# neggles/neurosis

Hardware: AMD Instinct MI355X
Metric: train images/sec (node) SDXL 1024^2 (higher is better)
Workload: dtype bf16

## Files before the change

### include/neurosis_hip.h

```cpp
#ifndef NEUROSIS_HIP_H
#define NEUROSIS_HIP_H

#ifdef __cplusplus
extern "C" {
#endif

const char* nk_last_error(void);
int nk_abi_version(void);

int nk_linear_fwd(const void* x, const void* w, const float* bias, const void* residual, void* y,
                  int M, int N, int K, long ldx, long ldw, long ldr, long ldy, float alpha, void* stream);
int nk_linear_dgrad(const void* dy, const void* w, const void* dx_add, void* dx, int M, int N, int K,
                    long lddy, long ldw, long ldadd, long lddx, void* stream);
long nk_linear_fwd_geglu_ok(int M, int I, int K);
int nk_linear_fwd_geglu(const void* x, const void* w, const float* bias, void* u, void* h, int M, int I, int K, long ldx, long ldw, long ldu,
                        long ldh, void* stream);
int nk_linear_dgrad_geglu(const void* dy, const void* w, const void* u, void* du, int M, int N, int I, long lddy, long ldw, long ldu,
                          long lddu, void* stream);
int nk_linear_fwd_geglu_s(const void* x, const void* w, const float* bias, void* s, void* h, int M, int I, int K, long ldx, long ldw, long lds,
                          long ldh, void* stream);
int nk_linear_dgrad_geglu_s(const void* dy, const void* w, const void* s, void* du, int M, int N, int I, long lddy, long ldw, long lds,
                            long lddu, void* stream);
int nk_linear_wgrad(const void* dy, const void* x, float* dw, int M, int N, int K, long lddy, long ldx,
                    long lddw, int accumulate, void* stream);
int nk_linear_wgrad_bias(const void* dy, const void* x, float* dw, float* dbias, int M, int N, int K, long lddy, long ldx, long lddw,
                         int accumulate, void* stream);

int nk_gemm_sk_status(void);

int nk_health_status(void);
int nk_health_clear(void);
int nk_health_export(int* dst, void* stream);
int nk_health_import(const int* src, void* stream);
int nk_debug_raise_health(void* stream);
int nk_debug_stamp(unsigned long long* dst, void* stream);
int nk_debug_launch_log(int mode);
long nk_debug_launch_names(char* buf, long cap);
// ... 241 lines not shown
```

### neurosis_amd/csrc/gemm.hip

```cpp
#include "nk_common.h"
#include "nk_gemm.h"
#include "gemm_plan.h"

#define NTHREADS 256
#define KC_IMAGE_BYTES (128 * 128)
#define MC_ROW_BYTES (128 * 2 + 16)
#define MC_IMAGE_BYTES (BK * MC_ROW_BYTES)
#define OPND_BYTES MC_IMAGE_BYTES
#define STAGE_BYTES (2 * OPND_BYTES)
#define SMEM_BYTES (2 * STAGE_BYTES)

static_assert(SMEM_BYTES >= BM * CS_LD * 4, "epilogue staging must fit");

__device__ __forceinline__ bool is_kc(int mode) { return mode == OP_KC || mode == OP_KCG; }

__device__ __forceinline__ long gather_offset(const NkGather& g, int n, int bh, int bw, int kh, int kw,
                                              int c, bool& valid) {
  int hn = bh + kh * g.ks;
  int wn = bw + kw * g.ks;
  bool ok = (hn >= 0) & (wn >= 0);
  ok &= (((hn | wn) & g.need_even) == 0);
  const int sh = g.div >> 1;
  int h = hn >> sh, w = wn >> sh;
  ok &= (h < g.H) & (w < g.W);
// ... 1148 lines not shown
        for (int j = 0; j < NJ; ++j)
          acc[i][j] = __builtin_amdgcn_mfma_f32_16x16x32_bf16(bfr[j], af[i], acc[i][j], 0, 0, 0);
    }
  }
#pragma unroll
  for (int ib = 0; ib < MI / 4; ++ib)
#pragma unroll
    for (int half = 0; half < NJ / 2; ++half) {
      float4_t pair[4][2];
#pragma unroll
      for (int i = 0; i < 4; ++i) { pair[i][0] = acc[ib * 4 + i][2 * half]; pair[i][1] = acc[ib * 4 + i][2 * half + 1]; }
      reg_epilogue_64x32<0>(p, p.C, pair, m0 + wm * WM + ib * 64, n0 + wn * WN + half * 32, lane);
    }
}

template <int AMODE, int GEGLU = 0>
__global__ __launch_bounds__(512, 2) void nk_gemm_xl2g_kernel(const NkGemmParams p) {
  extern __shared__ __attribute__((aligned(16))) char smem[];
  const int tid = threadIdx.x, lane = tid & 63, wave = tid >> 6;
  const int wm = wave >> 2, wn = wave & 3;
  const int nwg = gridDim.x, bid = blockIdx.x;
  const int q8 = nwg >> 3, r8 = nwg & 7, xcd = bid & 7;
  const int wg = (xcd < r8 ? xcd * (q8 + 1) : r8 * (q8 + 1) + (xcd - r8) * q8) + (bid >> 3);
  const int ntn = (p.N + XL_BN - 1) / XL_BN, ntm = (p.M + XL_BM - 1) / XL_BM;
  constexpr int GM = 4;
  const int per_group = GM * ntn;
  const int group = wg / per_group;
  const int first_m = group * GM;
  const int gm = min(GM, ntm - first_m);
  const int in_group = wg - group * per_group;
  const int nt = in_group / gm;
  const int m0 = (first_m + (in_group - nt * gm)) * XL_BM, n0 = nt * XL_BN;
  const int kend = p.K, nk = (p.K + BK - 1) / BK;

  OperandDMA<AMODE, 2> a0, a1;
  OperandDMA<OP_KC, 2> b0, b1;
  a0.init(p.A, p.lda, p.M, m0, tid, p.ga);
  a1.init(p.A, p.lda, p.M, m0 + 128, tid, p.ga);
  if constexpr (GEGLU) {
    const int I = p.N >> 1, wv = tid >> 6;
    const int gb0 = wv, gb1 = 8 + wv;
    b0.init(p.B, p.ldb, p.N, ((gb0 & 1) ? I : 0) + (n0 >> 1) + (gb0 >> 1) * 16 - wv * 16, tid, p.gb);
    b1.init(p.B, p.ldb, p.N, ((gb1 & 1) ? I : 0) + (n0 >> 1) + (gb1 >> 1) * 16 - wv * 16, tid, p.gb);
  } else {
    b0.init(p.B, p.ldb, p.N, n0, tid, p.gb);
    b1.init(p.B, p.ldb, p.N, n0 + 128, tid, p.gb);
  }
  const int s0 = p.k_rotate ? (xcd * nk) >> 3 : 0;
  const int wrap_at = nk - s0;
  int na0 = 0, na1 = 0, nb0 = 0, nb1 = 0, ka0 = kend, ka1 = kend, kb0 = kend, kb1 = kend;
  a0.start(s0 * BK); a1.start(s0 * BK); b0.start(s0 * BK); b1.start(s0 * BK);
#define X2_NEXT(op, src, g, cnt, ke)                        \
  do {                                                      \
    op.next_sources(ke, src, g, p.tw);                      \
    if (++cnt == wrap_at) { op.start(0); ke = s0 * BK; }    \
  } while (0)
#define X2_ISSUE(op, img, g, cnt, ke)                       \
  do {                                                      \
    const bf16_t* s_[2];                                    \
    X2_NEXT(op, s_, g, cnt, ke);                            \
    op.fire(0, s_[0], img); op.fire(1, s_[1], img);         \
  } while (0)
  float4_t acc[8][4];
#pragma unroll
  for (int i = 0; i < 8; ++i)
#pragma unroll
    for (int j = 0; j < 4; ++j) acc[i][j] = (float4_t){0.f, 0.f, 0.f, 0.f};

  bf16x8_t ar[8], bc0[4], bc1[4];
  typedef __attribute__((address_space(3))) const char* lds_c;
  const unsigned lds0 = (unsigned)(size_t)(lds_c)smem;
  const unsigned x0 = (unsigned)(((lane >> 4) ^ (lane & 7)) << 4);
  const unsigned arow = lds0 + (unsigned)(wm * 128 + (lane & 15)) * 128u;
  const unsigned brow = lds0 + 32768u + (unsigned)(wn * 64 + (lane & 15)) * 128u;
  const unsigned a_k0 = arow + x0, a_k1 = arow + (x0 ^ 64u), b_k0 = brow + x0, b_k1 = brow + (x0 ^ 64u);
#define X2_RD1(f, addr, OFF) asm volatile("ds_read_b128 %0, %1 offset:%2" : "=v"(f) : "v"(addr), "n"((OFF)))
#define X2_RDA(half)                                                                                             \
  X2_RD1(ar[0], ca0, (half) * 8192); X2_RD1(ar[1], ca0, (half) * 8192 + 2048); X2_RD1(ar[2], ca0, (half) * 8192 + 4096);    \
  X2_RD1(ar[3], ca0, (half) * 8192 + 6144); X2_RD1(ar[4], ca1, (half) * 8192); X2_RD1(ar[5], ca1, (half) * 8192 + 2048);    \
  X2_RD1(ar[6], ca1, (half) * 8192 + 4096); X2_RD1(ar[7], ca1, (half) * 8192 + 6144)
#define X2_RDB(f, half)                                                                                          \
  X2_RD1(f[0], cb0, (half) * 4096); X2_RD1(f[1], cb0, (half) * 4096 + 2048); X2_RD1(f[2], cb1, (half) * 4096);              \
  X2_RD1(f[3], cb1, (half) * 4096 + 2048)
#define X2_BAR() __builtin_amdgcn_sched_barrier(0); __builtin_amdgcn_s_barrier(); __builtin_amdgcn_sched_barrier(0)
#define X2_MM(rb, cb, bf, PREP)                                                                                  \
  asm volatile("s_waitcnt lgkmcnt(0)" ::: "memory");                                                             \
  __builtin_amdgcn_sched_barrier(0);                                                                             \
  __builtin_amdgcn_s_setprio(1);                                                                                 \
  PREP;               \
  _Pragma("unroll") for (int ks = 0; ks < 2; ++ks)                                                               \
    _Pragma("unroll") for (int i = 0; i < 4; ++i)                                                                \
      _Pragma("unroll") for (int j = 0; j < 2; ++j)                                                              \
        acc[(rb) + i][(cb) + j] = __builtin_amdgcn_mfma_f32_16x16x32_bf16(bf[ks * 2 + j], ar[ks * 4 + i], acc[(rb) + i][(cb) + j], 0, 0, 0); \
  __builtin_amdgcn_s_setprio(0)

  const bf16_t* sa0[2];
  const bf16_t* sa1[2];
  const bf16_t* sb0[2];
  const bf16_t* sb1[2];
  if (nk > 0) {
    X2_ISSUE(a0, smem, p.ga, na0, ka0);
    X2_ISSUE(a1, smem + 16384, p.ga, na1, ka1);
    X2_ISSUE(b0, smem + 32768, p.gb, nb0, kb0);
    X2_ISSUE(b1, smem + 49152, p.gb, nb1, kb1);
    X2_ISSUE(b0, smem + XL_STAGE_BYTES + 32768, p.gb, nb0, kb0);
    X2_ISSUE(b1, smem + XL_STAGE_BYTES + 49152, p.gb, nb1, kb1);
    asm volatile("s_waitcnt vmcnt(4)" ::: "memory");
  }
  X2_NEXT(a1, sa1, p.ga, na1, ka1);
  X2_BAR();
  if (wm == 1) { X2_BAR(); }
  for (int t = 0; t < nk; ++t) {
    const unsigned so = (unsigned)(t & 1) * XL_STAGE_BYTES;
    char* cur = smem + so;
// ... 15 lines not shown
    X2_BAR();
    X2_RDA(1);
    X2_BAR();
    X2_MM(4, 2, bc1, X2_NEXT(b0, sb0, p.gb, nb0, kb0); X2_NEXT(b1, sb1, p.gb, nb1, kb1));
    X2_BAR();
    b0.fire(0, sb0[0], cur + 32768);
    b0.fire(1, sb0[1], cur + 32768);
    b1.fire(0, sb1[0], cur + 49152);
    b1.fire(1, sb1[1], cur + 49152);
    asm volatile("s_waitcnt vmcnt(4)" ::: "memory");
    X2_BAR();
    X2_MM(4, 0, bc0, X2_NEXT(a1, sa1, p.ga, na1, ka1));
    X2_BAR();
  }
  if (wm == 0) { X2_BAR(); }
  asm volatile("s_waitcnt vmcnt(0)" ::: "memory");
#undef X2_NEXT
#undef X2_ISSUE
#undef X2_RD1
#undef X2_RDA
#undef X2_RDB
#undef X2_BAR
#undef X2_MM
  if constexpr (GEGLU) {
    const int I = p.N >> 1;
    const int abase = (n0 >> 1) + wn * 32;
    const int cl = (lane >> 4) * 4;
    float4_t ba[2], bg[2];
#pragma unroll
    for (int q = 0; q < 2; ++q) {
      ba[q] = p.bias ? *(const float4_t*)(p.bias + abase + q * 16 + cl) : (float4_t){0.f, 0.f, 0.f, 0.f};
      bg[q] = p.bias ? *(const float4_t*)(p.bias + I + abase + q * 16 + cl) : (float4_t){0.f, 0.f, 0.f, 0.f};
    }
    NkGemmParams ph = p;
    ph.N = I; ph.ldc = p.ld_h; ph.bias = nullptr;
    NkGemmParams ps = p;
    ps.bias = nullptr;
#pragma unroll
    for (int ib = 0; ib < 2; ++ib) {
      float4_t pa[4][2], pg[4][2], phh[4][2];
#pragma unroll
      for (int i = 0; i < 4; ++i)
#pragma unroll
        for (int q = 0; q < 2; ++q) {
          pa[i][q] = acc[ib * 4 + i][2 * q];
          pg[i][q] = acc[ib * 4 + i][2 * q + 1];
#pragma unroll
          for (int r = 0; r < 4; ++r) {
            const float av = bf2f(f2bf(pa[i][q][r] + ba[q][r])), gv = bf2f(f2bf(pg[i][q][r] + bg[q][r]));
            float cdf, pdf;
            normal_cdf_pdf(gv, cdf, pdf);
            const float ge = gv * cdf;
            phh[i][q][r] = av * ge;
            if (p.geglu_save) {
              pa[i][q][r] = ge;
              pg[i][q][r] = av * (cdf + gv * pdf);
            }
          }
        }
      const int mb = m0 + wm * 128 + ib * 64;
      if (p.geglu_save) {
        reg_epilogue_64x32<0>(ps, p.C, pa, mb, abase, lane);
        reg_epilogue_64x32<0>(ps, p.C, pg, mb, I + abase, lane);
      } else {
        reg_epilogue_64x32<0>(p, p.C, pa, mb, abase, lane);
        reg_epilogue_64x32<0>(p, p.C, pg, mb, I + abase, lane);
      }
      reg_epilogue_64x32<0>(ph, p.geglu_h, phh, mb, abase, lane);
    }
    return;
  }
#pragma unroll
  for (int ib = 0; ib < 2; ++ib)
#pragma unroll
    for (int half = 0; half < 2; ++half) {
      float4_t pair[4][2];
#pragma unroll
      for (int i = 0; i < 4; ++i) { pair[i][0] = acc[ib * 4 + i][2 * half]; pair[i][1] = acc[ib * 4 + i][2 * half + 1]; }
      reg_epilogue_64x32<0>(p, p.C, pair, m0 + wm * 128 + ib * 64, n0 + wn * 64 + half * 32, lane);
    }
}

__global__ void nk_zero_f32_kernel(float* __restrict__ dst, size_t n);
#include "gemm_g2.h"
#include "gemm_w160.h"
#include "conv_halo.h"
#include "conv_wgrad_halo.h"

typedef void (*NkGemmKernel)(const NkGemmParams);
static int launch_plan(NkGemmKernel kern, const NkGemmPlan& pl, const NkGemmParams& p, hipStream_t stream) {
  nk_optin_lds((const void*)kern, pl.smem);
  hipLaunchKernelGGL(kern, dim3(pl.grid[0], pl.grid[1], pl.grid[2]), dim3(pl.block), pl.smem, stream, p);
  return nk_check_launch(pl.name);
}

// ... 100 lines not shown
  if (!p.nbatch) NK_CHECK_ARG(((uintptr_t)p.A & 15) == 0 && ((uintptr_t)p.B & 15) == 0 && ((uintptr_t)p.C & 15) == 0);
  for (int z = 0; z < p.nbatch; ++z) NK_CHECK_ARG(((uintptr_t)p.Ab[z] & 15) == 0 && ((uintptr_t)p.Bb[z] & 15) == 0 && ((uintptr_t)p.Cb[z] & 15) == 0);
  if (amode == OP_KC) NK_CHECK_ARG((p.K & 7) == 0 && (p.lda & 7) == 0);
  if (bmode == OP_KC) NK_CHECK_ARG((p.K & 7) == 0 && (p.ldb & 7) == 0);
  if (amode == OP_KCG) NK_CHECK_ARG((p.ga.C & 7) == 0);
  if (amode == OP_MC) NK_CHECK_ARG((p.M & 7) == 0 && (p.lda & 7) == 0);
  if (bmode == OP_MC) NK_CHECK_ARG((p.N & 7) == 0 && (p.ldb & 7) == 0);
  if (bmode == OP_MCT) NK_CHECK_ARG((p.N & 7) == 0 && (p.tw.co_stride & 7) == 0 && (p.tw.tap_stride & 7) == 0);
  if (bmode == OP_MCG) NK_CHECK_ARG((p.gb.C & 7) == 0);
  if (p.residual) NK_CHECK_ARG(((uintptr_t)p.residual & 15) == 0 && ((p.ldr & 7) == 0 || (p.N & 7) != 0));
  if (!out_f32) NK_CHECK_ARG((p.ldc & 7) == 0 || (p.N & 7) != 0);
  if (p.fRowsPerBatch.d == 0) p.fRowsPerBatch = make_fastdiv(1);

  if (p.dbias || (p.nbatch && p.dbias_b[0])) NK_CHECK_ARG(amode == OP_MC && out_f32);
  if (p.geglu_h) {
    NK_CHECK_ARG(amode == OP_KC && bmode == OP_KC && !out_f32 && !p.nbatch && (p.N & 255) == 0 && (p.ld_h & 7) == 0 && !p.rowvec && !p.residual && p.alpha == 1.0f);
    NK_CHECK_ARG(((uintptr_t)p.geglu_h & 15) == 0 && (!p.bias || ((uintptr_t)p.bias & 15) == 0));
  } else if (p.geglu_u) {
    NK_CHECK_ARG(amode == OP_KC && bmode == OP_MC && !out_f32 && !p.nbatch && (p.N & 7) == 0 && (p.ld_u & 7) == 0 && !p.bias && !p.rowvec && !p.residual);
  }

  const TileEnv env = tile_env();
  const NkGemmPlan pl = nk_gemm_plan(p, amode, bmode, out_f32, allow_splitk, env);
  if (pl.err) {
    nk_set_error(__FILE__, __LINE__, pl.err);
    return NK_ERR_ARG;
  }
  if (pl.zero_c) NK_CHECK_ARG(p.ldc == p.N);
  const int logging = nk_launch_log_mode();
  char line[192];
  if (logging) nk_plan_line(pl, line, sizeof(line));
  if (logging == 3) {
    nk_launch_log_add(pl.name, line);
    return NK_OK;
  }

  p.ksplit_len = pl.ksplit_len; p.accumulate = pl.accumulate; p.k_rotate = pl.k_rotate; p.group_m = pl.group_m; p.sk_chunked = pl.sk_chunked;
  if (pl.zero_c)
    if (int rc = zero_split_outputs(p, stream)) return rc;
  if (pl.family == NK_FAM_SK) {
    p.sk_debug = env.sk_debug;
    if (int rc = sk_prepare(p, stream)) return rc;
  }

  int rc;
  switch (pl.family) {
    case NK_FAM_HALO: rc = launch_plan(halo_kernel(pl), pl, p, stream); break;
    case NK_FAM_WGRAD_HALO: rc = launch_plan(pl.flag ? nk_conv3x3_wgrad_halo_kernel<1> : nk_conv3x3_wgrad_halo_kernel<0>, pl, p, stream); break;
    case NK_FAM_W160: rc = launch_plan(pl.bn == 160 ? nk_gemm_w160_kernel<160> : nk_gemm_w160_kernel<128>, pl, p, stream); break;
    case NK_FAM_RING64: rc = launch_plan(nk_gemm_ring64_kernel, pl, p, stream); break;
    case NK_FAM_XL: rc = launch_plan(nk_gemm_xl_kernel<OP_KCG, 64, 64>, pl, p, stream); break;
    case NK_FAM_XL2G: rc = launch_plan(pl.flag ? nk_gemm_xl2g_kernel<OP_KC, 1> : nk_gemm_xl2g_kernel<OP_KC, 0>, pl, p, stream); break;
    case NK_FAM_G2P:
      rc = with_modes(amode, bmode, out_f32, [&](auto m) {
        using M = decltype(m);
        if constexpr (M::B == OP_MCG) return (int)NK_ERR_ARG;
        else return launch_plan(pl.bn == 160 ? nk_gemm_g2p_kernel<M::A, M::B, M::F32, 160> : nk_gemm_g2p_kernel<M::A, M::B, M::F32, 128>, pl, p, stream);
      });
      break;
    case NK_FAM_SK:
      rc = with_modes(amode, bmode, out_f32, [&](auto m) { using M = decltype(m); return launch_plan(nk_gemm_sk_kernel<M::A, M::B, M::F32>, pl, p, stream); });
      break;
    case NK_FAM_RING:
      rc = with_modes(amode, bmode, out_f32, [&](auto m) { using M = decltype(m); return launch_plan(nk_gemm_ring_kernel<M::A, M::B, M::F32>, pl, p, stream); });
      break;
    case NK_FAM_DMA:
      rc = with_modes(amode, bmode, out_f32, [&](auto m) { using M = decltype(m); return launch_plan(nk_gemm_dma_kernel<M::A, M::B, M::F32, 8>, pl, p, stream); });
// ... 1 lines not shown
    default:
      nk_set_error(__FILE__, __LINE__, "the plan names no kernel");
      return NK_ERR_ARG;
  }
  if (logging) nk_launch_log_add(nullptr, line);
  return rc;
}

int nk_halo_tiles_per_image(const NkGemmParams& p, int* bn) {
  const NkGemmPlan pl = nk_gemm_plan(p, OP_KCG, OP_KC, 0, 0, tile_env());
  if (pl.err || pl.family != NK_FAM_HALO) return 0;
  if (bn) *bn = pl.bn;
  return pl.tiles_per_image;
}

int nk_geglu_fwd_fusable(const NkGemmParams& p) {
  if (p.N & 255) return 0;
  const NkGemmPlan pl = nk_gemm_plan(p, OP_KC, OP_KC, 0, 0, tile_env());
  return !pl.err && pl.family == NK_FAM_XL2G && pl.flag ? 1 : 0;
}
```

### neurosis_amd/csrc/gemm_plan.h

```cpp
#pragma once
#include "nk_gemm.h"
#include <stdio.h>
#include <stdlib.h>

enum { OP_KC = 0, OP_KCG = 1, OP_MC = 2, OP_MCT = 3, OP_MCG = 4 };

#define BM 128
#define BN 128
#define BK 64
#define GROUP_M 8
#define CS_LD 132
#define V2_OPND_BYTES 16384
#define V2_STAGE_BYTES (2 * V2_OPND_BYTES)
#define V2_SMEM_BYTES (BM * CS_LD * 4)
#define RING_NS 4
#define RING_SMEM_BYTES (RING_NS * V2_STAGE_BYTES)
#define SK_NT 512
#define SK_SMEM_BYTES (2 * V2_STAGE_BYTES)
#define SK_MAX_GRID 512
#define R64_NS 8
#define R64_OPND 8192
#define R64_STAGE (2 * R64_OPND)
#define R64_SMEM (R64_NS * R64_STAGE)
#define XL_BM 256
// ... 25 lines not shown
#define WH_SMEM (2 * WH_STAGE)
#define WH_BCO 128
#define WH_BCI 64

struct TileEnv {
  int xl;
  int g2;
  int sk;
  int sk_debug;
  int w160;
  int w160_split;
  int krot;
  int r64;
  int halo;
  int wgrad_halo;
};
static int env_int(const char* e, int unset) { return e ? atoi(e) : unset; }
static int env_not0(const char* e) { return !(e && e[0] == '0'); }
static TileEnv tile_env() {
  static const int xl = env_not0(getenv("NK_GEMM_XL"));
  TileEnv t;
  t.xl = xl;
  t.g2 = env_int(getenv("NK_GEMM_G2"), 1);
  t.sk = env_int(getenv("NK_GEMM_SK"), 4);
  t.sk_debug = env_int(getenv("NK_SK_DEBUG"), 0) & 2;
  t.w160 = env_int(getenv("NK_GEMM_W160"), 1);
  t.w160_split = env_int(getenv("NK_GEMM_W160_SPLIT"), 1);
  t.krot = env_int(getenv("NK_GEMM_KROT"), 1) != 0;
  t.r64 = env_not0(getenv("NK_GEMM_R64"));
  t.halo = env_not0(getenv("NK_CONV_HALO"));
  t.wgrad_halo = env_int(getenv("NK_CONV_WGRAD_HALO"), 1);
  return t;
}

enum NkFamily { NK_FAM_NONE = 0, NK_FAM_RING64, NK_FAM_G2P, NK_FAM_XL, NK_FAM_XL2G, NK_FAM_SK, NK_FAM_RING, NK_FAM_DMA, NK_FAM_W160, NK_FAM_HALO, NK_FAM_WGRAD_HALO };
struct NkGemmPlan {
  int family;
  int bn;
  int halo_rows;
  int flag;
  const char* name;
  unsigned grid[3];
  int block, smem;
  int splitk;
  int ksplit_len, accumulate, k_rotate, group_m, sk_chunked;
  bool zero_c, zero_dbias;
  int tiles_per_image;
  const char* err;
};

static void nk_plan_line(const NkGemmPlan& pl, char* buf, size_t cap) {
  snprintf(buf, cap, "%s grid=%u,%u,%u %d %d %d %d %d %d %d %d %d", pl.name, pl.grid[0], pl.grid[1], pl.grid[2], pl.block, pl.smem, pl.splitk,
           pl.ksplit_len, pl.accumulate, (pl.zero_c ? 1 : 0) | (pl.zero_dbias ? 2 : 0), pl.k_rotate, pl.group_m, pl.sk_chunked);
}

static int cdiv(long a, long b) { return (int)((a + b - 1) / b); }
static int nbatch1(const NkGemmParams& p) { return p.nbatch ? p.nbatch : 1; }
static bool has_dbias(const NkGemmParams& p) {
  bool any = p.dbias != nullptr;
  for (int z = 0; z < p.nbatch && z < NK_MAX_BATCH; ++z) any = any || p.dbias_b[z] != nullptr;
  return any;
}

static bool k_rotate_on(const TileEnv& env, int k_len) { return env.krot && (k_len + BK - 1) / BK >= 8; }

static bool use_xl(const TileEnv& env, const NkGemmParams& p, int amode, int bmode, int out_f32, int splitk) {
  if (!env.xl || p.nbatch || out_f32 || splitk != 1 || bmode != OP_KC || !(amode == OP_KC || amode == OP_KCG)) return false;
  const long ntn = (p.N + XL_BN - 1) / XL_BN;
  const long tiles = (long)((p.M + XL_BM - 1) / XL_BM) * ntn;
  const long rounds = (tiles + 255) / 256;
  return tiles >= 224 && tiles * 10 >= rounds * 256 * 8 && ntn * XL_BN * 100 <= (long)p.N * 112 && p.K >= 4 * BK;
}

static bool halo_shape_ok(const NkGemmParams& p) {
  const NkGather& g = p.ga;
  if (!p.halo_nb || g.KW != 3 || p.K != 9 * g.C || g.rs != 1 || g.ks != 1 || g.div != 1 || g.off_h != -1 || g.off_w != -1) return false;
  if (g.Ho != g.H || g.Wo != g.W || (g.C & 63) || p.alpha != 1.0f || p.nbatch) return false;
  if (p.N % 160 && p.N % 128) return false;
  if ((p.N & 7) || (p.ldc & 7) || (p.residual && (p.ldr & 7))) return false;
  return true;
}
static int halo_bn(int N) { return N % 160 == 0 ? 160 : 128; }
static int halo_tile_rows(const NkGemmParams& p) {
  const NkGather& g = p.ga;
  const int bn = halo_bn(p.N);
  const long txn = (g.W + CH_TW - 1) / CH_TW;
// ... 148 lines not shown
}
static void plan_split(NkGemmPlan& pl, const NkGemmParams& p, int splits) {
  pl.splitk = splits;
  pl.ksplit_len = cdiv(cdiv(p.K, BK), splits) * BK;
  if (splits > 1 && pl.accumulate == 0) {
    pl.zero_c = true; pl.zero_dbias = has_dbias(p);
    pl.accumulate = 1;
  } else if (pl.accumulate == 2) {
    pl.accumulate = splits > 1 ? 1 : 0;
  }
}
static void plan_xl(NkGemmPlan& pl, const TileEnv& env, const NkGemmParams& p, int amode) {
  const long tiles = (long)cdiv(p.M, XL_BM) * cdiv(p.N, XL_BN);
  if (amode == OP_KC) {
    pl.flag = p.geglu_h != nullptr;
    plan_kernel(pl, NK_FAM_XL2G, pl.flag ? "nk_gemm_xl2g_kernel<geglu=1>" : "nk_gemm_xl2g_kernel<geglu=0>", tiles, 1, 1, 512, XL_SMEM_BYTES);
    pl.k_rotate = k_rotate_on(env, p.K);
  } else {
    plan_kernel(pl, NK_FAM_XL, "nk_gemm_xl_kernel", tiles, 1, 1, 1024, XL_SMEM_BYTES);
  }
}
static void plan_ring_or_dma(NkGemmPlan& pl, const TileEnv& env, const NkGemmParams& p) {
  const int ntm = cdiv(p.M, BM), ntn = cdiv(p.N, BN);
  {
    int per_xcd = (ntm * ntn + 7) / 8, g = 1;
    while ((g + 1) * (g + 1) <= per_xcd) ++g;
    pl.group_m = g > GROUP_M ? GROUP_M : g;
  }
  pl.k_rotate = k_rotate_on(env, pl.splitk > 1 ? pl.ksplit_len : p.K);
  if (!p.nbatch && (long)ntm * ntn * pl.splitk <= 256) plan_kernel(pl, NK_FAM_RING, "nk_gemm_ring_kernel", ntm * ntn, pl.splitk, 1, 512, RING_SMEM_BYTES);
  else plan_kernel(pl, NK_FAM_DMA, "nk_gemm_dma_kernel", ntm * ntn, pl.splitk, nbatch1(p), 512, V2_SMEM_BYTES);
}
static const char* halo_name(int bn, int rows, int stats) {
  static const char* const names[2][2][2] = {
      {{"nk_conv3x3_halo_kernel<128,4,stats=0>", "nk_conv3x3_halo_kernel<128,4,stats=1>"}, {"nk_conv3x3_halo_kernel<128,8,stats=0>", "nk_conv3x3_halo_kernel<128,8,stats=1>"}},
      {{"nk_conv3x3_halo_kernel<160,4,stats=0>", "nk_conv3x3_halo_kernel<160,4,stats=1>"}, {"nk_conv3x3_halo_kernel<160,8,stats=0>", "nk_conv3x3_halo_kernel<160,8,stats=1>"}}};
  return names[bn == 160][rows == 8][stats != 0];
}

static NkGemmPlan nk_gemm_plan(const NkGemmParams& p, int amode, int bmode, int out_f32, int allow_splitk, const TileEnv& env) {
  NkGemmPlan pl = {};
  pl.splitk = 1;
  pl.ksplit_len = p.ksplit_len; pl.accumulate = p.accumulate; pl.k_rotate = p.k_rotate; pl.group_m = p.group_m; pl.sk_chunked = p.sk_chunked;

  if (p.geglu_h) {
    if (amode != OP_KC || !use_xl(env, p, amode, bmode, out_f32, 1)) {
      pl.err = "fused GEGLU forward on a shape the 256 x 256 kernel does not take (ask nk_linear_fwd_geglu_ok first)";
      return pl;
    }
    plan_split(pl, p, 1);
    plan_xl(pl, env, p, OP_KC);
    return pl;
  }
  if (p.geglu_u) {
    plan_split(pl, p, 1);
    plan_ring_or_dma(pl, env, p);
    return pl;
  }
  if (use_halo(env, p, amode, bmode, out_f32)) {
    const NkGather& g = p.ga;
    pl.bn = halo_bn(p.N); pl.halo_rows = halo_tile_rows(p); pl.flag = p.stats_part != nullptr;
// ... 73 lines not shown
```

### neurosis_amd/csrc/nk_gemm.h

```cpp
#pragma once
#include "nk_common.h"

struct NkGather {
  int H, W, C;
  int Ho, Wo;
  int KW;
  int rs, ks;
  int off_h, off_w;
  int div;
  int need_even;
  FastDiv fWo, fHoWo, fC, fKW;
};

struct NkTapW {
  long co_stride, tap_stride;
  FastDiv fCout;
};

struct NkGemmParams {
  const bf16_t* A;
  const bf16_t* B;
  long lda, ldb;
  int M, N, K;
  NkGather ga, gb;
// ... 15 lines not shown
  int k_rotate;
  int nbatch;
  const bf16_t* Ab[8];
  const bf16_t* Bb[8];
  void* Cb[8];
  unsigned* sk_flags;
  float* sk_ws;
  unsigned* sk_health;
  float* dbias;
  float* dbias_b[8];
  const bf16_t* geglu_u;
  long ld_u;
  bf16_t* geglu_h;
  long ld_h;
  int geglu_save;
  int halo_nb;
  float* stats_part;
  int stats_groups;
};
#define NK_MAX_BATCH 8

enum { NK_OP_KC = 0, NK_OP_KCG = 1, NK_OP_MC = 2, NK_OP_MCT = 3, NK_OP_MCG = 4 };

int nk_gemm_dispatch(NkGemmParams& p, int amode, int bmode, int out_f32, int allow_splitk, hipStream_t stream);
int nk_halo_tiles_per_image(const NkGemmParams& p, int* bn);
int nk_geglu_fwd_fusable(const NkGemmParams& p);
```

### neurosis_amd/csrc/ops_gemm.hip

```cpp
#include "../../include/neurosis_hip.h"
#include "nk_gemm.h"
#include <string.h>

static NkGemmParams zero_params() {
  NkGemmParams p;
  memset(&p, 0, sizeof(p));
  p.alpha = 1.0f;
  p.fRowsPerBatch = make_fastdiv(1);
  p.ga.fWo = p.ga.fHoWo = p.ga.fC = p.ga.fKW = make_fastdiv(1);
  p.gb.fWo = p.gb.fHoWo = p.gb.fC = p.gb.fKW = make_fastdiv(1);
  p.tw.fCout = make_fastdiv(1);
  return p;
}

extern "C" int nk_linear_fwd(const void* x, const void* w, const float* bias, const void* residual, void* y,
                             int M, int N, int K, long ldx, long ldw, long ldr, long ldy, float alpha,
                             void* stream) {
  NkGemmParams p = zero_params();
  p.A = (const bf16_t*)x; p.lda = ldx;
  p.B = (const bf16_t*)w; p.ldb = ldw;
  p.M = M; p.N = N; p.K = K;
  p.C = y; p.ldc = ldy;
  p.bias = bias;
  p.residual = (const bf16_t*)residual; p.ldr = ldr;
// ... 29 lines not shown
  return nk_gemm_dispatch(p, NK_OP_KC, NK_OP_MC, 0, 0, (hipStream_t)stream);
}

static NkGemmParams geglu_fwd_params(const void* x, const void* w, const float* bias, void* u, void* h, int M, int I, int K, long ldx, long ldw,
                                      long ldu, long ldh) {
  NkGemmParams p = zero_params();
  p.A = (const bf16_t*)x; p.lda = ldx;
  p.B = (const bf16_t*)w; p.ldb = ldw;
  p.M = M; p.N = 2 * I; p.K = K;
  p.C = u; p.ldc = ldu;
  p.bias = bias;
  p.geglu_h = (bf16_t*)h; p.ld_h = ldh;
  return p;
}
extern "C" long nk_linear_fwd_geglu_ok(int M, int I, int K) {
  if (M <= 0 || I <= 0 || K <= 0 || (I & 127) || (K & 7)) return 0;
  NkGemmParams p = geglu_fwd_params(nullptr, nullptr, nullptr, nullptr, (void*)16, M, I, K, K, K, 2l * I, I);
  return nk_geglu_fwd_fusable(p);
}
extern "C" int nk_linear_fwd_geglu(const void* x, const void* w, const float* bias, void* u, void* h, int M, int I, int K, long ldx, long ldw,
                                   long ldu, long ldh, void* stream) {
  NK_CHECK_ARG(x && w && u && h && M > 0 && I > 0 && K > 0);
  NkGemmParams p = geglu_fwd_params(x, w, bias, u, h, M, I, K, ldx, ldw, ldu, ldh);
  return nk_gemm_dispatch(p, NK_OP_KC, NK_OP_KC, 0, 0, (hipStream_t)stream);
}

extern "C" int nk_linear_fwd_geglu_s(const void* x, const void* w, const float* bias, void* s, void* h, int M, int I, int K, long ldx, long ldw,
                                     long lds, long ldh, void* stream) {
  NK_CHECK_ARG(x && w && s && h && M > 0 && I > 0 && K > 0);
  NkGemmParams p = geglu_fwd_params(x, w, bias, s, h, M, I, K, ldx, ldw, lds, ldh);
  p.geglu_save = 1;
// ... 202 lines not shown
```

### neurosis_amd/lib.py

```python
from __future__ import annotations

import ctypes as C
import os
from pathlib import Path

import torch

CSRC = Path(__file__).resolve().parent / "csrc"
LIB_PATH = CSRC / "libneurosis_hip.so"

vp, i32, i64, f32 = C.c_void_p, C.c_int, C.c_long, C.c_float


class NkConvDesc(C.Structure):
    _fields_ = [(n, i32) for n in ("N", "H", "W", "Cin", "Cout", "KH", "KW", "stride", "pad_t", "pad_l", "Ho", "Wo", "upsample")]


class NkAttnDesc(C.Structure):
    _fields_ = (
        [(n, i32) for n in ("B", "H", "Lq", "Lk", "D")]
        + [(n, i64) for n in ("sq", "sk", "sv", "so", "bq", "bk", "bv", "bo", "sdq", "sdk", "sdv", "sdo", "bdq", "bdk", "bdv", "bdo")]
        + [("scale", f32), ("causal", i32)]
    )

# ... 3 lines not shown

class NkColpartBatch(C.Structure):
    _fields_ = [("part", vp * NK_COLPART_MAX), ("dgamma", vp * NK_COLPART_MAX), ("dbeta", vp * NK_COLPART_MAX), ("nrows", i32 * NK_COLPART_MAX),
                ("C", i32 * NK_COLPART_MAX), ("accumulate", i32 * NK_COLPART_MAX), ("n", i32)]


cdp, adp = C.POINTER(NkConvDesc), C.POINTER(NkAttnDesc)

SIGNATURES: dict[str, list] = {
    "nk_linear_fwd": [vp, vp, vp, vp, vp, i32, i32, i32, i64, i64, i64, i64, f32, vp],
    "nk_linear_dgrad": [vp, vp, vp, vp, i32, i32, i32, i64, i64, i64, i64, vp],
    "nk_linear_dgrad_geglu": [vp, vp, vp, vp, i32, i32, i32, i64, i64, i64, i64, vp],
    "nk_linear_fwd_geglu": [vp, vp, vp, vp, vp, i32, i32, i32, i64, i64, i64, i64, vp],
    "nk_linear_fwd_geglu_s": [vp, vp, vp, vp, vp, i32, i32, i32, i64, i64, i64, i64, vp],
    "nk_linear_dgrad_geglu_s": [vp, vp, vp, vp, i32, i32, i32, i64, i64, i64, i64, vp],
    "nk_linear_wgrad": [vp, vp, vp, i32, i32, i32, i64, i64, i64, i32, vp],
    "nk_linear_fwd_batched": [C.POINTER(vp), C.POINTER(vp), C.POINTER(vp), i32, i32, i32, i32, i64, i64, i64, vp],
    "nk_linear_wgrad_batched": [C.POINTER(vp), C.POINTER(vp), C.POINTER(vp), C.POINTER(vp), i32, i32, i32, i32, i64, i64, i64, i32, vp],
    "nk_linear_wgrad_bias": [vp, vp, vp, vp, i32, i32, i32, i64, i64, i64, i32, vp],
    "nk_conv2d_wgrad_bias": [cdp, vp, vp, vp, vp, i32, vp],
    "nk_conv2d_fwd": [cdp, vp, vp, vp, vp, vp, vp, vp],
    "nk_conv2d_fwd_stats": [cdp, vp, vp, vp, vp, vp, vp, vp, i32, vp],
    "nk_conv_weight_flip": [vp, vp, i32, i32, i32, vp],
    "nk_conv3x3_few_channels_fwd": [vp, vp, vp, vp, i32, i32, i32, i32, i32, vp],
    "nk_conv2d_dgrad": [cdp, vp, vp, vp, vp],
    "nk_conv2d_dgrad_flipped": [cdp, vp, vp, vp, vp],
    "nk_conv2d_wgrad": [cdp, vp, vp, vp, i32, vp],
    "nk_attention_fwd": [adp, vp, vp, vp, vp, vp, vp],
    "nk_attention_bwd": [adp, vp, vp, vp, vp, vp, vp, vp, vp, vp, vp, vp],
    "nk_attention_bwd_causal": [adp, vp, vp, vp, vp, vp, vp, vp, vp, vp, vp],
# ... 86 lines not shown
    "nk_conv2d_dgrad_flipped_ok": [cdp],
    "nk_linear_fwd_geglu_ok": [i32, i32, i32],
    "nk_layernorm_ws_floats": [i32, i32],
    "nk_layernorm_part_rows": [i32],
    "nk_colsum_ws_floats": [i64, i32],
    "nk_batchnorm_ws_floats": [i64, i32],
    "nk_lpips_layer_ws_floats": [i32, i32],
    "nk_attention_bwd_ws_floats": [adp],
    "nk_vq_search_ws_floats": [i64, i32],
    "nk_vq_quantize_ws_floats": [i64],
    "nk_resample_ws_floats": [i64, i32, i32, i32, i32],
    "nk_adafactor_tensor_bytes": [],
    "nk_came_tensor_bytes": [],
    "nk_adamw8bit_tensor_bytes": [],
    "nk_gemm_sk_status": [],
    "nk_health_status": [],
    "nk_debug_launch_names": [C.c_char_p, i64],
}

_lib = None


class NkError(RuntimeError):
    pass


def load() -> C.CDLL:
    global _lib
    if _lib is not None:
        return _lib
# ... 12 lines not shown
        fn = getattr(lib, name)
        fn.argtypes = argtypes
        fn.restype = i32
    for name, argtypes in SIZE_QUERIES.items():
        fn = getattr(lib, name)
        fn.argtypes = argtypes
        fn.restype = i64
    _lib = lib
    return lib


def launch_log(mode: int) -> None:
    call("nk_debug_launch_log", int(mode))


def launched() -> list[str]:
    buf = C.create_string_buffer(8192)
    n = query("nk_debug_launch_names", buf, len(buf))
    if n < 0:
        raise NkError("nk_debug_launch_names failed")
    return buf.value.decode().split("\n")[:-1]


def query(name: str, *args) -> int:
    return int(getattr(load(), name)(*args))


def call(name: str, *args) -> None:
    lib = load()
    rc = getattr(lib, name)(*args)
# ... 3 lines not shown
```

### neurosis_amd/models/diffusion.py

```python
from __future__ import annotations

import os
from contextlib import contextmanager, nullcontext
from math import ceil
from typing import Callable, Optional

import torch
from torch import Tensor, nn

from .. import ops
from ..modules.diffusion import Denoiser, DiffusionLoss, OpenAIWrapper, UNetModel
from ..nn import FlatParamStore
from .autoencoder import AutoencoderKL


class PrecomputedConditioner(nn.Module):

    def forward(self, batch: dict, force_zero_embeddings=None) -> dict:
        zeroed = set(force_zero_embeddings or ())
        out = {}
        for k in ("crossattn", "vector", "concat"):
            if k in batch and batch[k] is not None:
                out[k] = torch.zeros_like(batch[k]) if k in zeroed else batch[k]
        return out
# ... 80 lines not shown
        tr = self.trainable_embedders()
        if not tr:
            return
        for e in tr:
            if not hasattr(e, "trained_parameters"):
                raise NotImplementedError(f"trainable embedder {type(e).__name__}: only the CLIP text towers have a training chain")
        if self.stream_optimizer:
            raise NotImplementedError("stream_optimizer (the update streamed block by block behind backward) does not drive the text towers' groups")
        import torch.distributed as dist

        if dist.is_available() and dist.is_initialized() and dist.get_world_size() > 1:
            raise NotImplementedError("trainable text towers at world size > 1: their gradient exchange is not built (one GPU only)")

    def setup_flat_params(self) -> FlatParamStore:
        self._check_trainable_embedders()
        self.store = FlatParamStore([p for p in self.model.diffusion_model.parameters() if p.requires_grad])
        self.embedder_stores = []
        for e in self.trainable_embedders():
            st = FlatParamStore(e.trained_parameters())
            st.state.assume_zeroed = False
            self.embedder_stores.append(st)
        self.store.state.assume_zeroed = False
        if self.store.master.is_cuda:
            self.store.state.wgrad_stream = torch.cuda.Stream(device=self.store.master.device)
        if self.use_ema:
            self.configure_ema(self.ema_decay_rate)
        if self.optimizer is not None and self._torch_optimizer is None:
            self.configure_optimizers()
        self.stream_optimizer = self.stream_optimizer
        return self.store
# ... 313 lines not shown
```

### neurosis_amd/ops.py

```python
from __future__ import annotations

import ctypes as C
import os
import threading
import weakref
from dataclasses import dataclass
from typing import Callable, Optional

import torch
from torch import Tensor

from . import lib
from .lib import NkAttnDesc, NkConvDesc, call, query

BF16 = torch.bfloat16


class EngineState:

    _live = weakref.WeakSet()

    def __init__(self, wgrad_stream=None):
        self.grad_accumulate = False
        self.assume_zeroed = False
# ... 393 lines not shown
    _check2d(dy, "dy")
    M, N = dy.shape
    ws = _ws(query("nk_colsum_ws_floats", M, N), dy.device)
    call("nk_colsum", dy.data_ptr(), out.data_ptr(), ws.data_ptr(), M, N, dy.stride(0), int(accumulate), _stream())


def linear_fwd(x: Tensor, weight: Tensor, bias: Optional[Tensor], residual: Optional[Tensor] = None, need_dx: bool = True, x_saved=None):
    y = gemm_nt(x, w2d(weight), bias, residual)
    return y, _linear_bwd(x if x_saved is None else x_saved, weight, bias, need_dx)


def geglu_save_enabled() -> bool:
    return os.environ.get("NK_GEGLU_SAVE", "1") != "0"


def linear_geglu_fwd(x: Tensor, weight: Tensor, bias: Optional[Tensor], x_saved=None, save_derivative: bool = False):
    _check2d(x, "x")
    M, K = x.shape
    I2 = weight.shape[0]
    I = I2 // 2
    wq = w2d(weight)
    if I2 % 2 == 0 and x.is_contiguous() and query("nk_linear_fwd_geglu_ok", M, I, K):
        u = torch.empty(M, I2, dtype=BF16, device=x.device)
        h = torch.empty(M, I, dtype=BF16, device=x.device)
        call("nk_linear_fwd_geglu_s" if save_derivative else "nk_linear_fwd_geglu", x.data_ptr(), wq.data_ptr(), _p(bias), u.data_ptr(), h.data_ptr(), M, I, K,
             x.stride(0), wq.stride(0), u.stride(0), h.stride(0), _stream())
    else:
        u = gemm_nt(x, wq, bias, None)
        if save_derivative:
            h = torch.empty(M, I, dtype=BF16, device=x.device)
            call("nk_geglu_fwd_s", u.data_ptr(), h.data_ptr(), u.data_ptr(), M, I, _stream())
        else:
            h = geglu_fwd(u)[0]
    return u, h, _linear_bwd(x if x_saved is None else x_saved, weight, bias, True)


def _linear_bwd(x_in, weight: Tensor, bias: Optional[Tensor], need_dx: bool):
    def bwd(dy: Tensor, dx_add: Optional[Tensor] = None, geglu_u: Optional[Tensor] = None, geglu_s: Optional[Tensor] = None):
        entry = "nk_linear_dgrad_geglu"
        if geglu_s is not None:
            if geglu_u is not None:
# ... 855 lines not shown
```

Before: 25.90.

## Split GEGLU forward tail-wave tiles into half-width tiles to fill the last wave

```diff
diff --git a/include/neurosis_hip.h b/include/neurosis_hip.h
--- a/include/neurosis_hip.h
+++ b/include/neurosis_hip.h
@@ -21,6 +21,8 @@
                           long ldh, void* stream);
 int nk_linear_dgrad_geglu_s(const void* dy, const void* w, const void* s, void* du, int M, int N, int I, long lddy, long ldw, long lds,
                             long lddu, void* stream);
+int nk_gemm_tail_split(int on);
+long nk_gemm_tail_split_get(void);
 int nk_linear_wgrad(const void* dy, const void* x, float* dw, int M, int N, int K, long lddy, long ldx,
                     long lddw, int accumulate, void* stream);
 int nk_linear_wgrad_bias(const void* dy, const void* x, float* dw, float* dbias, int M, int N, int K, long lddy, long ldx, long lddw,
diff --git a/neurosis_amd/csrc/gemm.hip b/neurosis_amd/csrc/gemm.hip
--- a/neurosis_amd/csrc/gemm.hip
+++ b/neurosis_amd/csrc/gemm.hip
@@ -1186,14 +1186,12 @@
     }
 }
 
-template <int AMODE, int GEGLU = 0>
-__global__ __launch_bounds__(512, 2) void nk_gemm_xl2g_kernel(const NkGemmParams p) {
-  extern __shared__ __attribute__((aligned(16))) char smem[];
+template <int AMODE, int GEGLU, int HALF, int EDGE>
+__device__ __forceinline__ void xl2g_tile(const NkGemmParams& p, char* smem, const int wg, const int half, const int xcd) {
+  static_assert(!HALF || GEGLU, "the half-width tile exists for the fused GEGLU forward only");
   const int tid = threadIdx.x, lane = tid & 63, wave = tid >> 6;
-  const int wm = wave >> 2, wn = wave & 3;
-  const int nwg = gridDim.x, bid = blockIdx.x;
-  const int q8 = nwg >> 3, r8 = nwg & 7, xcd = bid & 7;
-  const int wg = (xcd < r8 ? xcd * (q8 + 1) : r8 * (q8 + 1) + (xcd - r8) * q8) + (bid >> 3);
+  const int wm = wave >> 2, wn = HALF ? (wave & 1) : (wave & 3);
+  const int wrow = HALF ? (wave >> 1) * 64 : wm * 128;
   const int ntn = (p.N + XL_BN - 1) / XL_BN, ntm = (p.M + XL_BM - 1) / XL_BM;
   constexpr int GM = 4;
   const int per_group = GM * ntn;
@@ -1204,6 +1202,10 @@
   const int nt = in_group / gm;
   const int m0 = (first_m + (in_group - nt * gm)) * XL_BM, n0 = nt * XL_BN;
   const int kend = p.K, nk = (p.K + BK - 1) / BK;
+  const int ac0 = (n0 >> 1) + half * 64;
+  if constexpr (HALF) {
+    if (ac0 >= (p.N >> 1)) return;
+  }
 
   OperandDMA<AMODE, 2> a0, a1;
   OperandDMA<OP_KC, 2> b0, b1;
@@ -1212,8 +1214,8 @@
   if constexpr (GEGLU) {
     const int I = p.N >> 1, wv = tid >> 6;
     const int gb0 = wv, gb1 = 8 + wv;
-    b0.init(p.B, p.ldb, p.N, ((gb0 & 1) ? I : 0) + (n0 >> 1) + (gb0 >> 1) * 16 - wv * 16, tid, p.gb);
-    b1.init(p.B, p.ldb, p.N, ((gb1 & 1) ? I : 0) + (n0 >> 1) + (gb1 >> 1) * 16 - wv * 16, tid, p.gb);
+    b0.init(p.B, p.ldb, p.N, ((gb0 & 1) ? I : 0) + ac0 + (gb0 >> 1) * 16 - wv * 16, tid, p.gb);
+    if constexpr (!HALF) b1.init(p.B, p.ldb, p.N, ((gb1 & 1) ? I : 0) + ac0 + (gb1 >> 1) * 16 - wv * 16, tid, p.gb);
   } else {
     b0.init(p.B, p.ldb, p.N, n0, tid, p.gb);
     b1.init(p.B, p.ldb, p.N, n0 + 128, tid, p.gb);
@@ -1221,7 +1223,8 @@
   const int s0 = p.k_rotate ? (xcd * nk) >> 3 : 0;
   const int wrap_at = nk - s0;
   int na0 = 0, na1 = 0, nb0 = 0, nb1 = 0, ka0 = kend, ka1 = kend, kb0 = kend, kb1 = kend;
-  a0.start(s0 * BK); a1.start(s0 * BK); b0.start(s0 * BK); b1.start(s0 * BK);
+  a0.start(s0 * BK); a1.start(s0 * BK); b0.start(s0 * BK);
+  if constexpr (!HALF) b1.start(s0 * BK);
 #define X2_NEXT(op, src, g, cnt, ke)                        \
   do {                                                      \
     op.next_sources(ke, src, g, p.tw);                      \
@@ -1233,9 +1236,10 @@
     X2_NEXT(op, s_, g, cnt, ke);                            \
     op.fire(0, s_[0], img); op.fire(1, s_[1], img);         \
   } while (0)
-  float4_t acc[8][4];
-#pragma unroll
-  for (int i = 0; i < 8; ++i)
+  constexpr int NRB = HALF ? 4 : 8;
+  float4_t acc[NRB][4];
+#pragma unroll
+  for (int i = 0; i < NRB; ++i)
 #pragma unroll
     for (int j = 0; j < 4; ++j) acc[i][j] = (float4_t){0.f, 0.f, 0.f, 0.f};
 
@@ -1243,7 +1247,7 @@
   typedef __attribute__((address_space(3))) const char* lds_c;
   const unsigned lds0 = (unsigned)(size_t)(lds_c)smem;
   const unsigned x0 = (unsigned)(((lane >> 4) ^ (lane & 7)) << 4);
-  const unsigned arow = lds0 + (unsigned)(wm * 128 + (lane & 15)) * 128u;
+  const unsigned arow = lds0 + (unsigned)(wrow + (lane & 15)) * 128u;
   const unsigned brow = lds0 + 32768u + (unsigned)(wn * 64 + (lane & 15)) * 128u;
   const unsigned a_k0 = arow + x0, a_k1 = arow + (x0 ^ 64u), b_k0 = brow + x0, b_k1 = brow + (x0 ^ 64u);
 #define X2_RD1(f, addr, OFF) asm volatile("ds_read_b128 %0, %1 offset:%2" : "=v"(f) : "v"(addr), "n"((OFF)))
@@ -1270,6 +1274,36 @@
   const bf16_t* sa1[2];
   const bf16_t* sb0[2];
   const bf16_t* sb1[2];
+  if constexpr (HALF) {
+    X2_ISSUE(a0, smem, p.ga, na0, ka0);
+    X2_ISSUE(a1, smem + 16384, p.ga, na1, ka1);
+    X2_ISSUE(b0, smem + 32768, p.gb, nb0, kb0);
+    X2_ISSUE(b0, smem + XL_STAGE_BYTES + 32768, p.gb, nb0, kb0);
+    X2_ISSUE(a0, smem + XL_STAGE_BYTES, p.ga, na0, ka0);
+    X2_ISSUE(a1, smem + XL_STAGE_BYTES + 16384, p.ga, na1, ka1);
+    asm volatile("s_waitcnt vmcnt(6)" ::: "memory");
+    X2_BAR();
+    if (wm == 1) { X2_BAR(); }
+    for (int t = 0; t < nk; ++t) {
+      const unsigned so = (unsigned)(t & 1) * XL_STAGE_BYTES, bo = so + (unsigned)((t >> 1) & 1) * 16384u;
+      char* cur = smem + so;
+      const unsigned ca0 = a_k0 + so, ca1 = a_k1 + so, cb0 = b_k0 + bo, cb1 = b_k1 + bo;
+      __builtin_amdgcn_sched_barrier(0);
+      X2_RDB(bc0, 0);
+      X2_RDA(0);
+      X2_BAR();
+      X2_MM(0, 0, bc0, X2_NEXT(b0, sb0, p.gb, nb0, kb0); X2_NEXT(a0, sa0, p.ga, na0, ka0); X2_NEXT(a1, sa1, p.ga, na1, ka1));
+      X2_BAR();
+      X2_RDB(bc1, 1);
+      b0.fire(0, sb0[0], smem + (bo ^ 16384u) + 32768);
+      b0.fire(1, sb0[1], smem + (bo ^ 16384u) + 32768);
+      asm volatile("s_waitcnt vmcnt(2)" ::: "memory");
+      X2_BAR();
+      X2_MM(0, 2, bc1, a0.fire(0, sa0[0], cur); a0.fire(1, sa0[1], cur); a1.fire(0, sa1[0], cur + 16384); a1.fire(1, sa1[1], cur + 16384));
+      X2_BAR();
+    }
+    if (wm == 0) { X2_BAR(); }
+  } else {
   if (nk > 0) {
     X2_ISSUE(a0, smem, p.ga, na0, ka0);
     X2_ISSUE(a1, smem + 16384, p.ga, na1, ka1);
@@ -1315,6 +1349,7 @@
     X2_BAR();
   }
   if (wm == 0) { X2_BAR(); }
+  }
   asm volatile("s_waitcnt vmcnt(0)" ::: "memory");
 #undef X2_NEXT
 #undef X2_ISSUE
@@ -1325,7 +1360,10 @@
 #undef X2_MM
   if constexpr (GEGLU) {
     const int I = p.N >> 1;
-    const int abase = (n0 >> 1) + wn * 32;
+    const int abase = ac0 + wn * 32;
+    if constexpr (EDGE) {
+      if (abase >= I) return;
+    }
     const int cl = (lane >> 4) * 4;
     float4_t ba[2], bg[2];
 #pragma unroll
@@ -1338,7 +1376,7 @@
     NkGemmParams ps = p;
     ps.bias = nullptr;
 #pragma unroll
-    for (int ib = 0; ib < 2; ++ib) {
+    for (int ib = 0; ib < NRB / 4; ++ib) {
       float4_t pa[4][2], pg[4][2], phh[4][2];
 #pragma unroll
       for (int i = 0; i < 4; ++i)
@@ -1359,7 +1397,7 @@
             }
           }
         }
-      const int mb = m0 + wm * 128 + ib * 64;
+      const int mb = m0 + wrow + ib * 64;
       if (p.geglu_save) {
         reg_epilogue_64x32<0>(ps, p.C, pa, mb, abase, lane);
         reg_epilogue_64x32<0>(ps, p.C, pg, mb, I + abase, lane);
@@ -1369,17 +1407,38 @@
       }
       reg_epilogue_64x32<0>(ph, p.geglu_h, phh, mb, abase, lane);
     }
-    return;
-  }
-#pragma unroll
-  for (int ib = 0; ib < 2; ++ib)
-#pragma unroll
-    for (int half = 0; half < 2; ++half) {
-      float4_t pair[4][2];
-#pragma unroll
-      for (int i = 0; i < 4; ++i) { pair[i][0] = acc[ib * 4 + i][2 * half]; pair[i][1] = acc[ib * 4 + i][2 * half + 1]; }
-      reg_epilogue_64x32<0>(p, p.C, pair, m0 + wm * 128 + ib * 64, n0 + wn * 64 + half * 32, lane);
-    }
+  } else {
+#pragma unroll
+    for (int ib = 0; ib < 2; ++ib)
+#pragma unroll
+      for (int hf = 0; hf < 2; ++hf) {
+        float4_t pair[4][2];
+#pragma unroll
+        for (int i = 0; i < 4; ++i) { pair[i][0] = acc[ib * 4 + i][2 * hf]; pair[i][1] = acc[ib * 4 + i][2 * hf + 1]; }
+        reg_epilogue_64x32<0>(p, p.C, pair, m0 + wm * 128 + ib * 64, n0 + wn * 64 + hf * 32, lane);
+      }
+  }
+}
+
+__device__ __forceinline__ int nk_xcd_order(int nwg, int bid) {
+  const int q8 = nwg >> 3, r8 = nwg & 7, x = bid & 7;
+  return (x < r8 ? x * (q8 + 1) : r8 * (q8 + 1) + (x - r8) * q8) + (bid >> 3);
+}
+
+template <int AMODE, int GEGLU = 0, int TAIL = 0>
+__global__ __launch_bounds__(512, 2) void nk_gemm_xl2g_kernel(const NkGemmParams p) {
+  extern __shared__ __attribute__((aligned(16))) char smem[];
+  static_assert(!TAIL || GEGLU, "the tail split exists for the fused GEGLU forward only");
+  const int bid = blockIdx.x, xcd = bid & 7;
+  const int nfull = TAIL ? (int)gridDim.x - p.tail_n : (int)gridDim.x;
+  if constexpr (TAIL) {
+    if (bid >= nfull) {
+      const int t = nk_xcd_order(p.tail_n, bid - nfull);
+      xl2g_tile<AMODE, 1, 1, 1>(p, smem, nfull + (t >> 1), t & 1, xcd);
+      return;
+    }
+  }
+  xl2g_tile<AMODE, GEGLU, 0, TAIL>(p, smem, nk_xcd_order(nfull, bid), 0, xcd);
 }
 
 __global__ void nk_zero_f32_kernel(float* __restrict__ dst, size_t n);
@@ -1510,7 +1569,7 @@
 
   if (p.dbias || (p.nbatch && p.dbias_b[0])) NK_CHECK_ARG(amode == OP_MC && out_f32);
   if (p.geglu_h) {
-    NK_CHECK_ARG(amode == OP_KC && bmode == OP_KC && !out_f32 && !p.nbatch && (p.N & 255) == 0 && (p.ld_h & 7) == 0 && !p.rowvec && !p.residual && p.alpha == 1.0f);
+    NK_CHECK_ARG(amode == OP_KC && bmode == OP_KC && !out_f32 && !p.nbatch && (p.N & 127) == 0 && (p.ld_h & 7) == 0 && !p.rowvec && !p.residual && p.alpha == 1.0f);
     NK_CHECK_ARG(((uintptr_t)p.geglu_h & 15) == 0 && (!p.bias || ((uintptr_t)p.bias & 15) == 0));
   } else if (p.geglu_u) {
     NK_CHECK_ARG(amode == OP_KC && bmode == OP_MC && !out_f32 && !p.nbatch && (p.N & 7) == 0 && (p.ld_u & 7) == 0 && !p.bias && !p.rowvec && !p.residual);
@@ -1532,6 +1591,7 @@
   }
 
   p.ksplit_len = pl.ksplit_len; p.accumulate = pl.accumulate; p.k_rotate = pl.k_rotate; p.group_m = pl.group_m; p.sk_chunked = pl.sk_chunked;
+  p.tail_n = pl.tail_n;
   if (pl.zero_c)
     if (int rc = zero_split_outputs(p, stream)) return rc;
   if (pl.family == NK_FAM_SK) {
@@ -1546,7 +1606,9 @@
     case NK_FAM_W160: rc = launch_plan(pl.bn == 160 ? nk_gemm_w160_kernel<160> : nk_gemm_w160_kernel<128>, pl, p, stream); break;
     case NK_FAM_RING64: rc = launch_plan(nk_gemm_ring64_kernel, pl, p, stream); break;
     case NK_FAM_XL: rc = launch_plan(nk_gemm_xl_kernel<OP_KCG, 64, 64>, pl, p, stream); break;
-    case NK_FAM_XL2G: rc = launch_plan(pl.flag ? nk_gemm_xl2g_kernel<OP_KC, 1> : nk_gemm_xl2g_kernel<OP_KC, 0>, pl, p, stream); break;
+    case NK_FAM_XL2G:
+      rc = launch_plan(pl.tail_kernel ? nk_gemm_xl2g_kernel<OP_KC, 1, 1> : pl.flag ? nk_gemm_xl2g_kernel<OP_KC, 1> : nk_gemm_xl2g_kernel<OP_KC, 0>, pl, p, stream);
+      break;
     case NK_FAM_G2P:
       rc = with_modes(amode, bmode, out_f32, [&](auto m) {
         using M = decltype(m);
@@ -1578,8 +1640,13 @@
   return pl.tiles_per_image;
 }
 
+extern "C" int nk_gemm_tail_split(int on) {
+  g_tile_tail_split = on;
+  return NK_OK;
+}
+extern "C" long nk_gemm_tail_split_get(void) { return tile_env().tail; }
+
 int nk_geglu_fwd_fusable(const NkGemmParams& p) {
-  if (p.N & 255) return 0;
   const NkGemmPlan pl = nk_gemm_plan(p, OP_KC, OP_KC, 0, 0, tile_env());
   return !pl.err && pl.family == NK_FAM_XL2G && pl.flag ? 1 : 0;
 }
diff --git a/neurosis_amd/csrc/gemm_plan.h b/neurosis_amd/csrc/gemm_plan.h
--- a/neurosis_amd/csrc/gemm_plan.h
+++ b/neurosis_amd/csrc/gemm_plan.h
@@ -63,7 +63,9 @@
   int r64;
   int halo;
   int wgrad_halo;
+  int tail;
 };
+static int g_tile_tail_split = 0;
 static int env_int(const char* e, int unset) { return e ? atoi(e) : unset; }
 static int env_not0(const char* e) { return !(e && e[0] == '0'); }
 static TileEnv tile_env() {
@@ -79,6 +81,7 @@
   t.r64 = env_not0(getenv("NK_GEMM_R64"));
   t.halo = env_not0(getenv("NK_CONV_HALO"));
   t.wgrad_halo = env_int(getenv("NK_CONV_WGRAD_HALO"), 1);
+  t.tail = env_not0(getenv("NK_GEMM_TAIL")) ? g_tile_tail_split : 0;
   return t;
 }
 
@@ -95,6 +98,8 @@
   int ksplit_len, accumulate, k_rotate, group_m, sk_chunked;
   bool zero_c, zero_dbias;
   int tiles_per_image;
+  int tail_first, tail_n;
+  bool tail_kernel;
   const char* err;
 };
 
@@ -119,6 +124,22 @@
   const long tiles = (long)((p.M + XL_BM - 1) / XL_BM) * ntn;
   const long rounds = (tiles + 255) / 256;
   return tiles >= 224 && tiles * 10 >= rounds * 256 * 8 && ntn * XL_BN * 100 <= (long)p.N * 112 && p.K >= 4 * BK;
+}
+
+struct TailSplit { long first; int n; };
+static TailSplit tail_split(const TileEnv& env, long tiles, int slots) {
+  if (env.tail < 0) {
+    const long first = -(long)env.tail - 1 < tiles ? -(long)env.tail - 1 : tiles;
+    return {first, (int)(2 * (tiles - first))};
+  }
+  const long rem = tiles % slots;
+  if (!env.tail || rem == 0 || 2 * rem > slots) return {tiles, 0};
+  return {tiles - rem, (int)(2 * rem)};
+}
+static bool use_xl_geglu(const TileEnv& env, const NkGemmParams& p, int amode, int bmode, int out_f32) {
+  if (amode != OP_KC) return false;
+  if (env.tail < 0) return env.xl && bmode == OP_KC && !p.nbatch && !out_f32 && (p.N & 127) == 0 && p.K >= 4 * BK;
+  return (p.N & 255) == 0 && use_xl(env, p, amode, bmode, out_f32, 1);
 }
 
 static bool halo_shape_ok(const NkGemmParams& p) {
@@ -297,7 +318,9 @@
   const long tiles = (long)cdiv(p.M, XL_BM) * cdiv(p.N, XL_BN);
   if (amode == OP_KC) {
     pl.flag = p.geglu_h != nullptr;
-    plan_kernel(pl, NK_FAM_XL2G, pl.flag ? "nk_gemm_xl2g_kernel<geglu=1>" : "nk_gemm_xl2g_kernel<geglu=0>", tiles, 1, 1, 512, XL_SMEM_BYTES);
+    const TailSplit ts = pl.flag ? tail_split(env, tiles, 256) : TailSplit{tiles, 0};
+    pl.tail_first = (int)ts.first; pl.tail_n = ts.n; pl.tail_kernel = ts.n > 0 || (pl.flag && env.tail < 0);
+    plan_kernel(pl, NK_FAM_XL2G, pl.flag ? "nk_gemm_xl2g_kernel<geglu=1>" : "nk_gemm_xl2g_kernel<geglu=0>", ts.first + ts.n, 1, 1, 512, XL_SMEM_BYTES);
     pl.k_rotate = k_rotate_on(env, p.K);
   } else {
     plan_kernel(pl, NK_FAM_XL, "nk_gemm_xl_kernel", tiles, 1, 1, 1024, XL_SMEM_BYTES);
@@ -327,7 +350,7 @@
   pl.ksplit_len = p.ksplit_len; pl.accumulate = p.accumulate; pl.k_rotate = p.k_rotate; pl.group_m = p.group_m; pl.sk_chunked = p.sk_chunked;
 
   if (p.geglu_h) {
-    if (amode != OP_KC || !use_xl(env, p, amode, bmode, out_f32, 1)) {
+    if (!use_xl_geglu(env, p, amode, bmode, out_f32)) {
       pl.err = "fused GEGLU forward on a shape the 256 x 256 kernel does not take (ask nk_linear_fwd_geglu_ok first)";
       return pl;
     }
diff --git a/neurosis_amd/csrc/nk_gemm.h b/neurosis_amd/csrc/nk_gemm.h
--- a/neurosis_amd/csrc/nk_gemm.h
+++ b/neurosis_amd/csrc/nk_gemm.h
@@ -53,6 +53,7 @@
   bf16_t* geglu_h;
   long ld_h;
   int geglu_save;
+  int tail_n;
   int halo_nb;
   float* stats_part;
   int stats_groups;
diff --git a/neurosis_amd/csrc/ops_gemm.hip b/neurosis_amd/csrc/ops_gemm.hip
--- a/neurosis_amd/csrc/ops_gemm.hip
+++ b/neurosis_amd/csrc/ops_gemm.hip
@@ -67,7 +67,7 @@
   return p;
 }
 extern "C" long nk_linear_fwd_geglu_ok(int M, int I, int K) {
-  if (M <= 0 || I <= 0 || K <= 0 || (I & 127) || (K & 7)) return 0;
+  if (M <= 0 || I <= 0 || K <= 0 || (I & 63) || (K & 7)) return 0;
   NkGemmParams p = geglu_fwd_params(nullptr, nullptr, nullptr, nullptr, (void*)16, M, I, K, K, K, 2l * I, I);
   return nk_geglu_fwd_fusable(p);
 }
diff --git a/neurosis_amd/lib.py b/neurosis_amd/lib.py
--- a/neurosis_amd/lib.py
+++ b/neurosis_amd/lib.py
@@ -41,6 +41,7 @@
     "nk_linear_fwd_geglu": [vp, vp, vp, vp, vp, i32, i32, i32, i64, i64, i64, i64, vp],
     "nk_linear_fwd_geglu_s": [vp, vp, vp, vp, vp, i32, i32, i32, i64, i64, i64, i64, vp],
     "nk_linear_dgrad_geglu_s": [vp, vp, vp, vp, i32, i32, i32, i64, i64, i64, i64, vp],
+    "nk_gemm_tail_split": [i32],
     "nk_linear_wgrad": [vp, vp, vp, i32, i32, i32, i64, i64, i64, i32, vp],
     "nk_linear_fwd_batched": [C.POINTER(vp), C.POINTER(vp), C.POINTER(vp), i32, i32, i32, i32, i64, i64, i64, vp],
     "nk_linear_wgrad_batched": [C.POINTER(vp), C.POINTER(vp), C.POINTER(vp), C.POINTER(vp), i32, i32, i32, i32, i64, i64, i64, i32, vp],
@@ -157,6 +158,7 @@
     "nk_came_tensor_bytes": [],
     "nk_adamw8bit_tensor_bytes": [],
     "nk_gemm_sk_status": [],
+    "nk_gemm_tail_split_get": [],
     "nk_health_status": [],
     "nk_debug_launch_names": [C.c_char_p, i64],
 }
@@ -199,6 +201,12 @@
     call("nk_debug_launch_log", int(mode))
 
 
+def gemm_tail_split(on: int | None = None) -> int:
+    if on is not None:
+        call("nk_gemm_tail_split", int(on))
+    return query("nk_gemm_tail_split_get")
+
+
 def launched() -> list[str]:
     buf = C.create_string_buffer(8192)
     n = query("nk_debug_launch_names", buf, len(buf))
diff --git a/neurosis_amd/models/diffusion.py b/neurosis_amd/models/diffusion.py
--- a/neurosis_amd/models/diffusion.py
+++ b/neurosis_amd/models/diffusion.py
@@ -118,6 +118,7 @@
 
     def setup_flat_params(self) -> FlatParamStore:
         self._check_trainable_embedders()
+        ops.geglu_tail_split(True)
         self.store = FlatParamStore([p for p in self.model.diffusion_model.parameters() if p.requires_grad])
         self.embedder_stores = []
         for e in self.trainable_embedders():
diff --git a/neurosis_amd/ops.py b/neurosis_amd/ops.py
--- a/neurosis_amd/ops.py
+++ b/neurosis_amd/ops.py
@@ -431,6 +431,16 @@
     return os.environ.get("NK_GEGLU_SAVE", "1") != "0"
 
 
+_geglu_tail_split = False
+
+
+def geglu_tail_split(on: Optional[bool] = None) -> bool:
+    global _geglu_tail_split
+    if on is not None:
+        _geglu_tail_split = bool(on)
+    return _geglu_tail_split
+
+
 def linear_geglu_fwd(x: Tensor, weight: Tensor, bias: Optional[Tensor], x_saved=None, save_derivative: bool = False):
     _check2d(x, "x")
     M, K = x.shape
@@ -440,8 +450,15 @@
     if I2 % 2 == 0 and x.is_contiguous() and query("nk_linear_fwd_geglu_ok", M, I, K):
         u = torch.empty(M, I2, dtype=BF16, device=x.device)
         h = torch.empty(M, I, dtype=BF16, device=x.device)
-        call("nk_linear_fwd_geglu_s" if save_derivative else "nk_linear_fwd_geglu", x.data_ptr(), wq.data_ptr(), _p(bias), u.data_ptr(), h.data_ptr(), M, I, K,
-             x.stride(0), wq.stride(0), u.stride(0), h.stride(0), _stream())
+        tail = _geglu_tail_split and lib.gemm_tail_split() == 0
+        if tail:
+            lib.gemm_tail_split(1)
+        try:
+            call("nk_linear_fwd_geglu_s" if save_derivative else "nk_linear_fwd_geglu", x.data_ptr(), wq.data_ptr(), _p(bias), u.data_ptr(), h.data_ptr(), M, I, K,
+                 x.stride(0), wq.stride(0), u.stride(0), h.stride(0), _stream())
+        finally:
+            if tail:
+                lib.gemm_tail_split(0)
     else:
         u = gemm_nt(x, wq, bias, None)
         if save_derivative:
```

After: 26.03, median of 6. Within noise of the previous version (+0.5%).
